# lizardfs/lizardfs

Hardware: NVIDIA H100
Metric: GiB/s encoded+CRC (ec(8,2), 64 MiB chunks) (higher is better)
Workload: dtype u8

## Files before the change

lizardfs_b200/csrc/fused.cu:

```cuda
#include <cuda.h>
#include <cuda_runtime.h>

#include <algorithm>
#include <cmath>
#include <numeric>
#include <cstdlib>
#include <cstring>
#include <memory>
#include <mutex>

#include "engine_internal.h"
#include "fused_kernel.cuh"
#include "convert_kernel.cuh"
#include "bs_recover_kernel.cuh"
#include "check_kernel.cuh"
#include "slices_kernel.cuh"
#include "recover_slices_kernel.cuh"
#include "host_math.h"

using namespace lzd;

typedef CUresult (*EncodeTiledFn)(CUtensorMap *, CUtensorMapDataType, cuuint32_t, void *, const cuuint64_t *, const cuuint64_t *,
                                  const cuuint32_t *, const cuuint32_t *, CUtensorMapInterleave, CUtensorMapSwizzle,
                                  CUtensorMapL2promotion, CUtensorMapFloatOOBfill);
// ... 62 lines not shown

static void set_raid6_pair(CoefPlanes *w, int x0, int x1) {
	const uint8_t g0 = gf_pow2(x0);
	coef_planes_set(w[0], g0);
	coef_planes_set(w[1], lz::gf_inv_host(g0 ^ gf_pow2(x1)));
}

static void elim3_constants(int x0, int x1, int x2, uint8_t c[6]) {
	const uint8_t A = gf_pow2(x0), pp = A ^ gf_pow2(x1), qq = A ^ gf_pow2(x2);
	c[0] = lz::gf_inv_host(lz::gf_mul_host(qq, pp ^ qq));
	c[1] = lz::gf_mul_host(pp, c[0]);
	c[2] = lz::gf_inv_host(pp);
	c[3] = lz::gf_mul_host(qq, c[2]);
	c[4] = A;
	c[5] = lz::gf_mul_host(A, A);
}

template <class... P, class... A>
static int launch(lzgpu_ctx *ctx, void (*kernel)(P...), const lzgpu_launch_geometry &geo, int per_sm, uint64_t units, cudaStream_t st,
                  const A &...args) {
	const int grid = persistent_grid(ctx, units, per_sm, geo);
	kernel<<<grid, geo.threads, geo.smem_bytes, st>>>(args...);
	CUDA_TRY(cudaGetLastError());
	ctx->stats.kernel_launches++;
	return LZGPU_OK;
}

template <class F>
static int set_smem(F *kernel, int bytes) {
	CUDA_TRY(cudaFuncSetAttribute(kernel, cudaFuncAttributeMaxDynamicSharedMemorySize, bytes));
	return LZGPU_OK;
}

using EncodeKernel = void (*)(CUtensorMap, FusedParams);
struct EncodeKernelEntry {
	int m;
	bool generic, striped, split, bs;
	uint32_t k, g;
	EncodeKernel fn;
	EncodeKernel narrow;
};
template <int M, bool GENERIC, int KT = 0, int GT = 0, bool STRIPED = false, bool SPLIT = false>
static EncodeKernelEntry encoder() {
	EncodeKernelEntry k{M, GENERIC, STRIPED, SPLIT, false, KT, GT, fused_stream_kernel<M, GENERIC, KT, GT, 64, STRIPED, SPLIT>, nullptr};
	if constexpr (GENERIC) k.narrow = fused_stream_kernel<M, GENERIC, KT, GT, 64, STRIPED, SPLIT, 1>;
	return k;
}
template <int M, int KT = 0, int GT = 0, bool STRIPED = false>
static EncodeKernelEntry bitsliced() {
	return {M, false, STRIPED, false, true, KT, GT, fused_stream_kernel<M, false, KT, GT, 64, STRIPED, false, 8>, nullptr};
}
static const EncodeKernelEntry kEncoders[] = {
	encoder<0, false>(), encoder<1, false>(), encoder<2, false>(), encoder<3, false>(), encoder<4, false>(),
	encoder<1, true>(), encoder<2, true>(), encoder<3, true>(), encoder<4, true>(),
	encoder<1, false, 0, 0, false, true>(), encoder<2, false, 0, 0, false, true>(), encoder<3, false, 0, 0, false, true>(),
	encoder<4, false, 0, 0, false, true>(), encoder<4, true, 0, 0, false, true>(),
	encoder<1, false, 0, 0, true>(), encoder<2, false, 0, 0, true>(), encoder<3, false, 0, 0, true>(), encoder<4, false, 0, 0, true>(),
	encoder<4, true, 0, 0, true>(),
	encoder<2, false, 8, 7>(),
	encoder<1, false, 2, 32>(),
	encoder<1, false, 3, 20>(),
	encoder<2, false, 3, 16>(),
	encoder<2, false, 4, 12>(),
	encoder<2, false, 6, 9>(),
	encoder<3, false, 5, 8>(),
	encoder<3, false, 6, 8>(),
	encoder<4, false, 8, 8>(),
	encoder<3, false, 8, 6>(),
	encoder<1, false, 4, 16>(),
	encoder<2, false, 5, 10>(),
	encoder<2, false, 10, 5>(),
	encoder<3, false, 4, 8>(),
	encoder<4, false, 10, 6>(),
	encoder<4, false, 12, 5>(),
	encoder<4, false, 6, 8>(),
	encoder<4, false, 4, 8>(),
	encoder<2, false, 8, 7, true>(), encoder<1, false, 2, 32, true>(), encoder<1, false, 3, 20, true>(), encoder<2, false, 3, 16, true>(),
	encoder<3, false, 5, 8, true>(), encoder<4, false, 8, 8, true>(),
	bitsliced<3>(), bitsliced<4>(), bitsliced<3, 0, 0, true>(), bitsliced<4, 0, 0, true>(),
	bitsliced<4, 8, 8>(), bitsliced<4, 10, 6>(), bitsliced<4, 12, 5>(), bitsliced<4, 6, 8>(), bitsliced<4, 4, 8>(),
	bitsliced<3, 8, 8>(), bitsliced<3, 9, 6>(), bitsliced<3, 10, 6>(), bitsliced<3, 12, 5>(), bitsliced<4, 8, 8, true>(),
};

static const EncodeKernelEntry *find_encoder(int M, bool generic, uint32_t K, uint32_t G, bool striped, bool split, bool bs) {
	const EncodeKernelEntry *runtime_k = nullptr;
	for (const EncodeKernelEntry &k : kEncoders) {
		if (k.m != M || k.generic != generic || k.striped != striped || k.split != split || k.bs != bs) continue;
		if (k.k == K && k.g == G) return &k;
		if (k.k == 0) runtime_k = &k;
	}
	return runtime_k;
}

using RecoverKernel = void (*)(TmapArray, RecoverParams);
struct RecoverKernelEntry {
	int kernel;
	uint32_t e, kt;
	bool first_e, wide;
	RecoverKernel fn;
};
template <int GEO, int E, int KT, int R0 = -1, int R1 = -1>
static RecoverKernelEntry recoverer() {
	constexpr int kernel = GEO == 2 ? LZGPU_KERNEL_RECOVER_GEO2 : GEO == 1 ? LZGPU_KERNEL_RECOVER_GEO1 : LZGPU_KERNEL_RECOVER_GEO0;
	return {kernel, E, KT, R0 == 0, false, fused_recover_kernel<E, KT, R0, R1, 64, GEO>};
}
template <int E, bool WIDE>
static RecoverKernelEntry direct() {
	return {LZGPU_KERNEL_RECOVER_DIRECT, E, 0, false, WIDE, fused_recover_kernel<E, 0, kRecoverDirect, -1, 64, 2, WIDE ? direct_wide_words(E) : 1>};
}
static const RecoverKernelEntry kRecoverers[] = {
	recoverer<0, 1, 8, 0>(), recoverer<1, 1, 8, 0>(), recoverer<2, 1, 8, 0>(),
	recoverer<0, 1, 0, 0>(), recoverer<1, 1, 0, 0>(), recoverer<2, 1, 0, 0>(),
	recoverer<0, 1, 0>(), recoverer<1, 1, 0>(), recoverer<2, 1, 0>(),
	recoverer<0, 2, 8, 0, 1>(), recoverer<1, 2, 8, 0, 1>(), recoverer<2, 2, 8, 0, 1>(),
	recoverer<0, 2, 0, 0, 1>(), recoverer<1, 2, 0, 0, 1>(), recoverer<2, 2, 0, 0, 1>(),
	recoverer<0, 2, 0>(), recoverer<1, 2, 0>(), recoverer<2, 2, 0>(),
	recoverer<0, 3, 0, 0, 1>(), recoverer<2, 3, 0, 0, 1>(), recoverer<0, 3, 0>(), recoverer<2, 3, 0>(),
	recoverer<0, 4, 0, 0, 1>(), recoverer<2, 4, 0, 0, 1>(), recoverer<0, 4, 0>(), recoverer<2, 4, 0>(),
	recoverer<2, 1, 3, 0>(), recoverer<2, 2, 3, 0, 1>(), recoverer<2, 2, 4, 0, 1>(), recoverer<2, 2, 5, 0, 1>(),
	recoverer<2, 3, 5, 0, 1>(), recoverer<2, 2, 6, 0, 1>(), recoverer<2, 3, 6, 0, 1>(),
// ... 128 lines not shown
}

void lz_fused_destroy(lzgpu_ctx *ctx) {
	if (ctx->fused && ctx->fused->d_sm_ctr) cudaFree(ctx->fused->d_sm_ctr);
	delete ctx->fused;
	ctx->fused = nullptr;
}

extern "C" int lzgpu_debug_last_launch(lzgpu_ctx *ctx, uint32_t *grid, uint32_t *units) {
	if (!ctx || !ctx->fused || !grid || !units) return LZGPU_ERR_ARG;
	std::lock_guard<std::mutex> lock(ctx->fused->last_mu);
	*grid = ctx->fused->last_geo.grid;
	*units = ctx->fused->last_geo.units;
	return LZGPU_OK;
}

extern "C" int lzgpu_debug_last_geometry(lzgpu_ctx *ctx, lzgpu_launch_geometry *out) {
	if (!ctx || !ctx->fused || !out) return LZGPU_ERR_ARG;
	std::lock_guard<std::mutex> lock(ctx->fused->last_mu);
	*out = ctx->fused->last_geo;
	return LZGPU_OK;
}

static CUresult make_tensor_map(const FusedState *fs, CUtensorMap *map, const void *base, uint64_t rows_per_chunk, uint64_t n_chunks,
                                uint64_t chunk_stride, uint32_t box_rows) {
	const cuuint64_t dims[3] = {static_cast<cuuint64_t>(kRowBytes), rows_per_chunk, n_chunks};
	const cuuint64_t strides[2] = {static_cast<cuuint64_t>(kRowBytes), chunk_stride ? chunk_stride : rows_per_chunk * kRowBytes};
	const cuuint32_t box[3] = {kStepBytes, box_rows, 1};
	const cuuint32_t estr[3] = {1, 1, 1};
	return fs->encode_tiled(map, CU_TENSOR_MAP_DATA_TYPE_UINT8, 3, const_cast<void *>(base), dims, strides, box, estr, CU_TENSOR_MAP_INTERLEAVE_NONE,
	                        CU_TENSOR_MAP_SWIZZLE_128B, static_cast<CUtensorMapL2promotion>(fs->promo), CU_TENSOR_MAP_FLOAT_OOB_FILL_NONE);
}

static int fused_run(lzgpu_ctx *ctx, int M, bool generic, const uint8_t *coef_rows, uint32_t K, uint32_t n_chunks, uint32_t nb,
                     const void *d_data, size_t chunk_stride, void *d_parity, size_t parity_stride, void *d_crc, size_t crc_stride,
                     cudaStream_t st, void *const *split_out = nullptr, size_t split_stride = 0, uint32_t crc_row_base = 0, bool skip_data_crc = false,
                     int striped_policy = -2 ) {
	FusedState *fs = ctx->fused;
	const int spol = split_out ? 0 : (striped_policy == -2 ? fs->striped : striped_policy);
	FusedPlan pl;
	if (!split_out && fused_bitslice(M, generic, fs->bitslice, K))
		pl = fused_plan(M, generic, K, n_chunks, nb, chunk_stride, std::min(fs->max_smem, fs->bs_smem_cap), 64, spol, true, fs->bs_max_stages, fs->bs_max_gf_warps);
	if (!pl.ok) pl = fused_plan(M, generic, K, n_chunks, nb, chunk_stride, std::min(fs->max_smem, fused_smem_cap(M, generic, 64)), 64, spol);
	if (!pl.ok || (reinterpret_cast<uintptr_t>(d_data) % 16)) return LZGPU_NOT_HANDLED;
	const uint32_t G = pl.G;
	const bool flat = pl.mode == 1u, striped = pl.mode == 2u;
	FusedParams p{};
	p.parity = static_cast<uint8_t *>(d_parity);
	p.crc = static_cast<uint32_t *>(d_crc);
	p.tables = ctx->d_crc_tables;
	p.parity_stride = parity_stride;
	p.crc_stride = crc_stride;
	p.n_chunks = n_chunks;
	p.nb = nb;
	p.pb = pl.pb;
	p.K = K;
	p.G = G;
	p.n_stages = pl.n_stages;
	p.flat = pl.mode;
	p.flat_magic = (1ull << 40) / p.pb + 1;
	p.units_per_chunk = pl.units_per_chunk;
	p.total_units = pl.total_units;
	std::memcpy(p.qmult, fs->qmult, sizeof(p.qmult));
	p.zconst = lz::crc_of_zeros(LZGPU_BLOCK_SIZE);
	p.probe = fs->probe;
	p.evict_first = static_cast<uint32_t>(fs->evict_first);
	p.crc_row_base = crc_row_base;
	p.skip_data_crc = skip_data_crc ? 1u : 0u;
	if (generic) {
		for (int r = 0; r < M; ++r)
			for (uint32_t j = 0; j < K; ++j) {
				coef_planes_set(p.coef[r * 32 + j], coef_rows[r * K + j]);
			}
	}
	const uint64_t map_rows = flat ? static_cast<uint64_t>(n_chunks) * nb * 4 : static_cast<uint64_t>(nb) * 4, map_chunks = flat ? 1 : n_chunks;
	const uint64_t map_stride = flat ? 0 : chunk_stride;
	const uint32_t box_rows = striped ? K * 4 : G * K * 4;
	CUtensorMap map;
	const CUresult r = make_tensor_map(fs, &map, d_data, map_rows, map_chunks, map_stride, box_rows);
	if (r != CUDA_SUCCESS) {
		lz_set_error("cuTensorMapEncodeTiled failed with CUresult %d (rows/chunk %llu, chunks %llu, stride %llu, box rows %u)", static_cast<int>(r),
		             static_cast<unsigned long long>(map_rows), static_cast<unsigned long long>(map_chunks), static_cast<unsigned long long>(map_stride), box_rows);
		return LZGPU_ERR_CUDA;
	}
	if (split_out) {
		if (striped || (split_stride % 16)) return LZGPU_NOT_HANDLED;
		for (uint32_t j = 0; j < K; ++j) p.data_out[j] = static_cast<uint8_t *>(split_out[j]);
		for (int r = 0; r < M; ++r) p.par_out[r] = static_cast<uint8_t *>(split_out[K + r]);
		p.part_out_stride = split_stride;
	}
	const EncodeKernelEntry *k = find_encoder(M, generic, K, G, striped, split_out != nullptr, pl.bs);
	if (!k) return LZGPU_NOT_HANDLED;
	const lzgpu_launch_geometry geo = launch_geo(pl.bs ? LZGPU_KERNEL_ENCODE_BITSLICE : LZGPU_KERNEL_ENCODE, pl.threads, G, pl.n_stages,
	                                             pl.bs ? (16 * G + 31) / 32 : 0, pl.smem);
	const EncodeKernel fn = k->narrow && fused_generic_item_words(G) == 1 ? k->narrow : k->fn;
	return launch(ctx, fn, geo, fused_ctas_per_sm(M, generic, 64, pl.bs), p.total_units, st, map, p);
}

int lz_fused_encode(lzgpu_ctx *ctx, const lzgpu_goal *goal, uint32_t n_chunks, uint32_t nb, const void *d_data, size_t chunk_stride,
                    void *d_parity, size_t parity_stride, void *d_crc, size_t crc_stride, cudaStream_t st) {
	FusedState *fs = ctx->fused;
	if (!fs || fs->disabled) return LZGPU_NOT_HANDLED;
	const int K = goal->k, M = goal->m;
	if (lz::uses_cauchy(K, M)) {
		if (fs->cauchy_encode_off) return LZGPU_NOT_HANDLED;
		uint8_t gen[LZGPU_MAX_PARTS * LZGPU_MAX_DATA];
		lz::rs_generator(K, M, gen);
		if (M == 4) return fused_run(ctx, 4, true, gen + K * K, K, n_chunks, nb, d_data, chunk_stride, d_parity, parity_stride, d_crc, crc_stride, st);
		const uint32_t pb = (nb + K - 1) / K;
		for (int rows : {4, M % 4})
			if (rows && !fused_plan(rows, true, K, n_chunks, nb, chunk_stride, std::min(fs->max_smem, fused_smem_cap(rows, true, 64)), 64, 0).ok) return LZGPU_NOT_HANDLED;
		if (reinterpret_cast<uintptr_t>(d_data) % 16) return LZGPU_NOT_HANDLED;
		for (int r0 = 0; r0 < M; r0 += 4) {
			int rc = fused_run(ctx, std::min(4, M - r0), true, gen + (K + r0) * K, K, n_chunks, nb, d_data, chunk_stride,
			                   static_cast<uint8_t *>(d_parity) + static_cast<size_t>(r0) * pb * LZGPU_BLOCK_SIZE, parity_stride, d_crc, crc_stride, st, nullptr, 0,
			                   static_cast<uint32_t>(r0), r0 > 0, 0);
			if (rc != LZGPU_OK) return rc == LZGPU_NOT_HANDLED ? LZGPU_ERR_CUDA : rc;
		}
		return LZGPU_OK;
	}
	if (M > 4) return LZGPU_NOT_HANDLED;
	int rc = fused_run(ctx, M, false, nullptr, K, n_chunks, nb, d_data, chunk_stride, d_parity, parity_stride, d_crc, crc_stride, st);
	if (rc == LZGPU_NOT_HANDLED && goal->kind == LZGPU_KIND_EC) {
		uint8_t gen[LZGPU_MAX_PARTS * LZGPU_MAX_DATA];
		lz::rs_generator(K, M, gen);
		rc = fused_run(ctx, M, true, gen + K * K, K, n_chunks, nb, d_data, chunk_stride, d_parity, parity_stride, d_crc, crc_stride, st, nullptr, 0, 0, false, 0);
	}
	return rc;
}
// ... 462 lines not shown
```

lizardfs_b200/csrc/fused_kernel.cuh:

```cuda
#pragma once
#include <cuda.h>

#include "bitslice.cuh"
#include "device_math.cuh"
#include "fused_plan.h"

namespace lzd {

#ifdef LZ_ENABLE_PROBE
#define LZ_PROBE(bit) (p.probe & (bit))
#else
#define LZ_PROBE(bit) 0
#endif

#ifdef LZ_ALL_LANES_ARRIVE
#define LZ_RING_ARRIVERS 32u
#define LZ_RING_LANE(lane) true
#else
#define LZ_RING_ARRIVERS 1u
#define LZ_RING_LANE(lane) ((lane) == 0)
#endif

struct FusedParams {
	uint8_t *parity;
// ... 45 lines not shown
	return false;
}
__device__ __forceinline__ void mbar_expect_tx(uint32_t bar, uint32_t bytes) {
	asm volatile("mbarrier.arrive.expect_tx.shared::cta.b64 _, [%0], %1;" ::"r"(bar), "r"(bytes) : "memory");
}
__device__ __forceinline__ void mbar_wait(uint32_t addr, uint32_t parity) {
	uint32_t done;
	do {
		asm volatile(
		    "{\n\t.reg .pred p;\n\t"
		    "mbarrier.try_wait.parity.shared::cta.b64 p, [%1], %2, %3;\n\t"
		    "selp.u32 %0, 1, 0, p;\n\t}"
		    : "=r"(done)
		    : "r"(addr), "r"(parity), "r"(0x989680u)
		    : "memory");
	} while (!done);
}
__device__ __forceinline__ void tma_load_3d_evict_first(uint32_t smem_dst, const CUtensorMap *map, int c0, int c1, int c2, uint32_t bar) {
	uint64_t policy;
	asm volatile("createpolicy.fractional.L2::evict_first.b64 %0, 1.0;" : "=l"(policy));
	asm volatile(
	    "cp.async.bulk.tensor.3d.shared::cluster.global.tile.mbarrier::complete_tx::bytes.L2::cache_hint [%0], [%1, {%2, %3, %4}], [%5], %6;" ::"r"(
	        smem_dst),
	    "l"(reinterpret_cast<uint64_t>(map)), "r"(c0), "r"(c1), "r"(c2), "r"(bar), "l"(policy)
	    : "memory");
}
__device__ __forceinline__ void tma_load_3d(uint32_t smem_dst, const CUtensorMap *map, int c0, int c1, int c2, uint32_t bar) {
	asm volatile(
	    "cp.async.bulk.tensor.3d.shared::cluster.global.tile.mbarrier::complete_tx::bytes [%0], [%1, {%2, %3, %4}], [%5];" ::"r"(
	        smem_dst),
	    "l"(reinterpret_cast<uint64_t>(map)), "r"(c0), "r"(c1), "r"(c2), "r"(bar)
	    : "memory");
}

template <int FW>
struct FoldSpec;
template <>
struct FoldSpec<64> {
	static constexpr int deg = 53, nlag = 9;
	__host__ __device__ static constexpr int lag(int t) { return t == 0 ? 15 : t == 1 ? 17 : t == 2 ? 20 : t == 3 ? 23 : t == 4 ? 26 : t == 5 ? 28 : t == 6 ? 46 : t == 7 ? 50 : 53; }
};

__device__ __forceinline__ uint4 lds128(uint32_t addr) {
	uint4 v;
	asm volatile("ld.shared.v4.u32 {%0,%1,%2,%3}, [%4];" : "=r"(v.x), "=r"(v.y), "=r"(v.z), "=r"(v.w) : "r"(addr));
	return v;
}
__device__ __forceinline__ void sts128(uint32_t addr, const uint4 &v) {
	asm volatile("st.shared.v4.u32 [%0], {%1,%2,%3,%4};" ::"r"(addr), "r"(v.x), "r"(v.y), "r"(v.z), "r"(v.w) : "memory");
}

template <int W>
__device__ __forceinline__ void lds_item(uint32_t addr, uint32_t (&v)[W]) {
	if constexpr (W == 4) asm volatile("ld.shared.v4.u32 {%0,%1,%2,%3}, [%4];" : "=r"(v[0]), "=r"(v[1]), "=r"(v[2]), "=r"(v[3]) : "r"(addr));
	else if constexpr (W == 2) asm volatile("ld.shared.v2.u32 {%0,%1}, [%2];" : "=r"(v[0]), "=r"(v[1]) : "r"(addr));
	else asm volatile("ld.shared.u32 %0, [%1];" : "=r"(v[0]) : "r"(addr));
}
template <int W>
__device__ __forceinline__ void sts_item(uint32_t addr, const uint32_t (&v)[W]) {
	if constexpr (W == 4) asm volatile("st.shared.v4.u32 [%0], {%1,%2,%3,%4};" ::"r"(addr), "r"(v[0]), "r"(v[1]), "r"(v[2]), "r"(v[3]) : "memory");
	else if constexpr (W == 2) asm volatile("st.shared.v2.u32 [%0], {%1,%2};" ::"r"(addr), "r"(v[0]), "r"(v[1]) : "memory");
	else asm volatile("st.shared.u32 [%0], %1;" ::"r"(addr), "r"(v[0]) : "memory");
}
template <int W>
__device__ __forceinline__ void stg_item(void *p, const uint32_t (&v)[W]) {
	if constexpr (W == 4) asm volatile(LZ_STG ".v4.u32 [%0], {%1,%2,%3,%4};" ::"l"(p), "r"(v[0]), "r"(v[1]), "r"(v[2]), "r"(v[3]) : "memory");
// ... 25 lines not shown
		win[S & (FW - 1)] = acc;
	}
}

template <int FW, bool AUX = true>
__device__ __forceinline__ void fold_step(uint32_t (&win)[FW], FoldAux &aux, int base, uint32_t row_addr_swz) {
#pragma unroll
	for (int c = 0; c < 8; ++c) {
		const uint4 v = lds128(row_addr_swz ^ (c << 4));
		fold_word<FW, AUX>(win, aux, base + 4 * c + 0, v.x);
		fold_word<FW, AUX>(win, aux, base + 4 * c + 1, v.y);
		fold_word<FW, AUX>(win, aux, base + 4 * c + 2, v.z);
		fold_word<FW, AUX>(win, aux, base + 4 * c + 3, v.w);
	}
}

template <int FW>
__device__ __forceinline__ uint32_t fold_finish(uint32_t (&win)[FW], const uint32_t *tab) {
	constexpr int deg = FoldSpec<FW>::deg;
#pragma unroll
	for (int j = 0; j < deg; ++j) {
		uint32_t acc = 0;
#pragma unroll
		for (int t = 0; t < FoldSpec<FW>::nlag; ++t)
			if (FoldSpec<FW>::lag(t) > j) acc ^= win[(j - FoldSpec<FW>::lag(t)) & (FW - 1)];
		win[j] = acc;
	}
	uint32_t st = 0;
#pragma unroll
	for (int j = 0; j < deg; ++j) st = crc_step_word_ldg(st, win[j], tab);
	return st;
}

template <int M, bool GENERIC, int KT, int GT, int FW, bool STRIPED = false, bool SPLIT = false, int W = fused_item_words(M, GENERIC)>
__global__ void __launch_bounds__(fused_threads(M, GENERIC, W == 8), fused_ctas_per_sm(M, GENERIC, FW, W == 8))
fused_stream_kernel(const __grid_constant__ CUtensorMap tmap, const FusedParams p) {
	constexpr int kNSTc = fused_nst(FW, M, GENERIC, W == 8), kNPST = fused_npst(FW, M, GENERIC);
	const uint32_t kNST = (W == 8) ? p.n_stages : static_cast<uint32_t>(kNSTc);
	constexpr int NT = fused_threads(M, GENERIC, W == 8);
	constexpr int PC = (M == 0) ? 0 : (GENERIC ? M : M - 1);
	constexpr int P0 = GENERIC ? 0 : 1;
	constexpr bool BS = W == 8;
	static_assert(!BS || ((M == 3 || M == 4) && !GENERIC && !SPLIT && FW == 64), "bit-sliced items: three or four Vandermonde rows, plain encode");

	extern __shared__ __align__(1024) uint8_t smem[];
	const uint32_t sbase = smem_u32(smem);
	const uint32_t K = KT ? KT : p.K, G = GT ? GT : p.G;
	const uint32_t ROWS = G * K * 4;
	const uint32_t PROWS = G * PC * 4;
	const uint32_t stage_bytes = ROWS * kStepBytes;
	const uint32_t pstage_bytes = (PROWS * kStepBytes + 1023u) & ~1023u;
	const uint32_t pstage0 = sbase + kNST * stage_bytes;
	const uint32_t misc = pstage0 + kNPST * pstage_bytes;
	const uint32_t a_blk = misc;
	const uint32_t a_full = misc + 520, a_empty = a_full + 8 * kNST, a_pfull = a_empty + 8 * kNST, a_pempty = a_pfull + 8 * kNPST;

	const uint32_t tid = threadIdx.x;
	const uint32_t warp = tid >> 5, lane = tid & 31;
	constexpr uint32_t CPI = 32 / W;
	const uint32_t n_items = 4 * CPI * G * (M > 0 ? 1 : 0);
	const uint32_t n_gf_warps = (min(n_items, (uint32_t)NT) + 31) / 32;
	const uint32_t bs_gf_warps = BS ? n_gf_warps : 0, bs_gf_warp0 = NT / 32 - bs_gf_warps;
	const uint32_t first_pwarp = ROWS / 32, last_pwarp = PROWS ? (ROWS + PROWS - 1) / 32 : 0;
	const uint32_t n_stage_warps = BS ? bs_gf_warps + (ROWS + 31) / 32 : max((ROWS + 31) / 32, n_gf_warps);

	const uint32_t my_units = blockIdx.x < p.total_units ? (p.total_units - blockIdx.x + gridDim.x - 1) / gridDim.x : 0;
	const uint32_t total_steps = my_units * kStepsPerUnit;

	auto issue_load = [&](uint32_t c, uint32_t gi, uint32_t step, uint32_t st) {
		mbar_expect_tx(a_full + 8 * st, stage_bytes);
		if (p.evict_first)
			tma_load_3d_evict_first(sbase + st * stage_bytes, &tmap, static_cast<int>(step * kStepBytes), static_cast<int>(gi * ROWS),
			                        static_cast<int>(c), a_full + 8 * st);
		else
			tma_load_3d(sbase + st * stage_bytes, &tmap, static_cast<int>(step * kStepBytes), static_cast<int>(gi * ROWS), static_cast<int>(c),
			            a_full + 8 * st);
	};

	auto issue_striped = [&](uint32_t unit, uint32_t step, uint32_t st, uint32_t first_g, uint32_t g_step) {
		const uint32_t s0 = unit * G;
		const uint32_t n_valid = min(G, p.n_chunks * p.pb - s0);
		const uint32_t stripe_bytes = K * 4 * kStepBytes;
		if (first_g == 0) mbar_expect_tx(a_full + 8 * st, n_valid * stripe_bytes);
		for (uint32_t g = first_g; g < n_valid; g += g_step) {
// ... 11 lines not shown
			s_out = sg - cc * p.pb;
		} else {
			c_out = unit_c;
			s_out = sg;
		}
	};
	const uint32_t stripes_total = p.flat ? p.n_chunks * p.pb : p.pb;

	if (tid == 0) {
		for (uint32_t s = 0; s < kNST; ++s) {
			mbar_init(a_full + 8 * s, 1);
			mbar_init(a_empty + 8 * s, n_stage_warps);
		}
		for (int s = 0; s < kNPST; ++s) {
			mbar_init(a_pfull + 8 * s, (n_gf_warps ? n_gf_warps : 1) * LZ_RING_ARRIVERS);
			mbar_init(a_pempty + 8 * s, (PROWS ? (last_pwarp - first_pwarp + 1) : 1) * LZ_RING_ARRIVERS);
		}
		asm volatile("fence.mbarrier_init.release.cluster;" ::: "memory");
		if (total_steps)
			for (uint32_t g0 = 0; g0 < kNST; ++g0) {
				if (STRIPED) issue_striped(blockIdx.x, g0, g0, 0, 1);
				else issue_load(blockIdx.x / p.units_per_chunk, blockIdx.x % p.units_per_chunk, g0, g0);
			}
	}
	__syncthreads();

	const uint32_t cw = warp;
	const uint32_t vt = tid;
	const bool is_data_row = vt < ROWS;
	const bool is_parity_row = vt >= ROWS && vt < ROWS + PROWS;
	const bool has_stream = is_data_row || is_parity_row;
	const uint32_t prow = vt - ROWS;
	const uint32_t my_row = is_data_row ? vt : prow;
	const uint32_t row_addr0 = ((is_data_row ? sbase : pstage0) + my_row * kStepBytes) ^ ((my_row & 7) << 4);
	const uint32_t row_stride = is_data_row ? stage_bytes : pstage_bytes;
	const bool warp_has_items = !BS && cw < n_gf_warps;
	const bool warp_has_prow = PROWS && cw >= first_pwarp && cw <= last_pwarp;
	const bool warp_reads_stage = BS ? cw < (ROWS + 31) / 32 : cw < n_stage_warps;

	if constexpr (BS) {
		if (cw >= bs_gf_warp0) {
			uint32_t it = 0, st = 0, ph = 0, pst = 0, pph = 0;
			const uint32_t item = tid - 32 * bs_gf_warp0;
			const bool has_item = item < n_items;
			const uint32_t col = item & 7, h = (item >> 3) & 1, g = item >> 4;
			const uint32_t rbase = g * K * 4 + h;
			const uint32_t a_even0 = (rbase * kStepBytes) ^ ((col ^ (rbase & 7)) << 4);
			for (uint32_t unit = blockIdx.x; unit < p.total_units; unit += gridDim.x) {
				const uint32_t c = unit / p.units_per_chunk, gi = unit % p.units_per_chunk;
				const uint32_t stripe0 = gi * G;
				const uint32_t next_unit = unit + gridDim.x;
				const uint32_t next_c = next_unit / p.units_per_chunk, next_gi = next_unit % p.units_per_chunk;
				const uint32_t sg = stripe0 + g;
				uint32_t pc = 0, stripe = 0;
				const bool live = has_item && sg < stripes_total;
				if (live) locate(sg, c, pc, stripe);
				uint8_t *const dst0 = p.parity + pc * p.parity_stride + (static_cast<unsigned long long>(stripe) << 16) + (h << 14) + col * 16;
				const unsigned long long part_bytes = static_cast<unsigned long long>(p.pb) * 65536ull;
				for (int step = 0; step < kStepsPerUnit; ++step) {
					const uint32_t stage = sbase + st * stage_bytes;
					const uint32_t pstage = pstage0 + pst * pstage_bytes;
					mbar_wait(a_full + 8 * st, ph);
					if (!LZ_PROBE(2)) {
						mbar_wait(a_pempty + 8 * pst, pph ^ 1);
						if (has_item) {
							BsRows<BS ? M : 4> rows4;
							bs_rows_clear(rows4);
// ... 35 lines not shown
						if (__shfl_sync(0xffffffffu, refill, 0)) {
							asm volatile("fence.proxy.async.shared::cta;" ::: "memory");
							if (step + kNST < kStepsPerUnit) issue_striped(unit, step + kNST, st, lane, 32);
							else issue_striped(next_unit, step + kNST - kStepsPerUnit, st, lane, 32);
						}
					} else if (lane == 0) {
						if (mbar_arrive_is_last(a_empty + 8 * st) && it + kNST < total_steps) {
							asm volatile("fence.proxy.async.shared::cta;" ::: "memory");
							if (step + kNST < kStepsPerUnit) issue_load(c, gi, step + kNST, st);
							else issue_load(next_c, next_gi, step + kNST - kStepsPerUnit, st);
						}
					}
					++it;
					if (++st == kNST) { st = 0; ph ^= 1; }
					if (++pst == kNPST) { pst = 0; pph ^= 1; }
				}
			}
			return;
		}
	}

	uint32_t win[FW];
	FoldAux aux;
	uint32_t it = 0;
	uint32_t st = 0, ph = 0;
	uint32_t pst = 0, pph = 0;
	uint32_t unit_parity = 0;

	for (uint32_t unit = blockIdx.x; unit < p.total_units; unit += gridDim.x, unit_parity ^= 1) {
		const uint32_t c = unit / p.units_per_chunk, gi = unit % p.units_per_chunk;
		const uint32_t stripe0 = gi * G;
		const uint32_t next_unit = unit + gridDim.x;
		const uint32_t next_c = next_unit / p.units_per_chunk, next_gi = next_unit % p.units_per_chunk;
#pragma unroll
		for (int i = 0; i < FW; ++i) win[i] = 0;
#pragma unroll
		for (int i = 0; i < 32; ++i) aux.y[i] = 0;

		for (int step0 = 0; step0 < kStepsPerUnit; step0 += FW / 32) {
#pragma unroll
			for (int sub = 0; sub < FW / 32; ++sub) {
				const int step = step0 + sub;
				const uint32_t stage = sbase + st * stage_bytes;
				const uint32_t pstage = pstage0 + pst * pstage_bytes;
				if (warp_reads_stage) mbar_wait(a_full + 8 * st, ph);

				if (!BS && M > 0 && warp_has_items && !LZ_PROBE(2)) {
					if (PC > 0) mbar_wait(a_pempty + 8 * pst, pph ^ 1);
					for (uint32_t item = vt; item < n_items; item += NT) {
						const uint32_t col = item % CPI, q = (item / CPI) & 3, g = item / (4 * CPI);
						const uint32_t c16 = (col * W) >> 2, sub = ((col * W) & 3) << 2;
						uint32_t acc[M > 0 ? M : 1][W];
#pragma unroll
						for (int r = 0; r < M; ++r)
#pragma unroll
							for (int w = 0; w < W; ++w) acc[r][w] = 0;
						const uint32_t rbase = g * K * 4 + q;
						const uint32_t sg = stripe0 + g;
						uint32_t pc = 0, stripe = 0;
						if (sg < stripes_total) locate(sg, c, pc, stripe);
						const unsigned long long in_part = (static_cast<unsigned long long>(stripe) << 16) + (q << 14) + step * kStepBytes + col * (4 * W);
						const uint32_t a_even = ((stage + rbase * kStepBytes) ^ ((c16 ^ (rbase & 7)) << 4)) + sub;
						const uint32_t a_odd = ((stage + rbase * kStepBytes) ^ ((c16 ^ ((rbase & 7) ^ 4)) << 4)) + sub;
#pragma unroll
						for (int j = static_cast<int>(K) - 1; j >= 0; --j) {
							uint32_t v[W];
							lds_item<W>(((j & 1) ? a_odd : a_even) + 4u * j * kStepBytes, v);
							if (SPLIT) {
								uint8_t *dp = p.data_out[j];
								if (dp && sg < stripes_total) stg_item<W>(dp + pc * p.part_out_stride + in_part, v);
							}
							if (GENERIC) {
#pragma unroll
								for (int r = 0; r < M; ++r) {
									const CoefPlanes &cp = p.coef[r * 32 + j];
#pragma unroll
									for (int w = 0; w < W; ++w) acc[r][w] = gf_mac<6>(acc[r][w], v[w], cp);
								}
							} else {
#pragma unroll
								for (int r = 0; r < M; ++r) {
#pragma unroll
									for (int w = 0; w < W; ++w) {
										const uint32_t a = acc[r][w], d = v[w];
										acc[r][w] = r == 0 ? (a ^ d) : r == 1 ? gf_x2_add(a, d) : r == 2 ? gf_x4_add(a, d) : gf_x8_add(a, d);
									}
								}
							}
						}
						if (sg < stripes_total && !LZ_PROBE(8)) {
							if (SPLIT) {
#pragma unroll
								for (int r = 0; r < M; ++r)
									if (p.par_out[r]) stg_item<W>(p.par_out[r] + pc * p.part_out_stride + in_part, acc[r]);
							} else {
								uint8_t *dst = p.parity + pc * p.parity_stride + in_part;
#pragma unroll
								for (int r = 0; r < M; ++r) stg_item<W>(dst + static_cast<unsigned long long>(r) * p.pb * 65536ull, acc[r]);
							}
						}
#pragma unroll
						for (int r = P0; r < M; ++r) {
							const uint32_t pr = (g * PC + (r - P0)) * 4 + q;
							sts_item<W>(((pstage + pr * kStepBytes) ^ ((c16 ^ (pr & 7)) << 4)) + sub, acc[r]);
						}
					}
					if (PC > 0) {
						__syncwarp();
						if (LZ_RING_LANE(lane)) mbar_arrive(a_pfull + 8 * pst);
					}
				}

				if (PC > 0 && warp_has_prow && !LZ_PROBE(2)) mbar_wait(a_pfull + 8 * pst, pph);
				if (has_stream && !(GENERIC && is_data_row && p.skip_data_crc) && !LZ_PROBE(4)) {
					const uint32_t rowp = row_addr0 + (is_data_row ? st : pst) * row_stride;
					fold_step<FW, (NT * fused_ctas_per_sm(M, GENERIC, FW, BS) <= 512)>(win, aux, sub * 32, rowp);
				}
				__syncwarp();
				if (STRIPED) {
					uint32_t refill = 0;
					if (lane == 0) refill = warp_reads_stage && mbar_arrive_is_last(a_empty + 8 * st) && it + kNST < total_steps;
					if (__shfl_sync(0xffffffffu, refill, 0)) {
						asm volatile("fence.proxy.async.shared::cta;" ::: "memory");
						if (step + kNST < kStepsPerUnit) issue_striped(unit, step + kNST, st, lane, 32);
						else issue_striped(next_unit, step + kNST - kStepsPerUnit, st, lane, 32);
					}
				} else if (lane == 0) {
					if (warp_reads_stage && mbar_arrive_is_last(a_empty + 8 * st) && it + kNST < total_steps) {
						asm volatile("fence.proxy.async.shared::cta;" ::: "memory");
						if (step + kNST < kStepsPerUnit) issue_load(c, gi, step + kNST, st);
						else issue_load(next_c, next_gi, step + kNST - kStepsPerUnit, st);
					}
				}
				if (PC > 0 && warp_has_prow && !LZ_PROBE(2) && LZ_RING_LANE(lane)) mbar_arrive(a_pempty + 8 * pst);
				++it;
				if (++st == kNST) { st = 0; ph ^= 1; }
				if (++pst == kNPST) { pst = 0; pph ^= 1; }
			}
		}

		uint32_t lin = 0;
		if (has_stream) lin = crc_mulmod(fold_finish<FW>(win, p.tables), p.qmult[my_row & 3]);
		lin ^= __shfl_xor_sync(0xffffffffu, lin, 1);
		lin ^= __shfl_xor_sync(0xffffffffu, lin, 2);
		const uint32_t blk = a_blk + unit_parity * 256;
		if (is_data_row && (vt & 3) == 0) {
			const uint32_t bl = vt >> 2;
			if (M > 0 && !GENERIC) asm volatile("st.shared.u32 [%0], %1;" ::"r"(blk + (vt & ~3u)), "r"(lin) : "memory");
			const uint32_t sg = stripe0 + bl / K;
			uint32_t bc, bs;
			locate(sg, c, bc, bs);
			const uint32_t b = bs * K + bl % K;
			if (sg < stripes_total && b < p.nb && !(GENERIC && p.skip_data_crc)) p.crc[bc * p.crc_stride + b] = lin ^ p.zconst;
		}
		if (is_parity_row && (prow & 3) == 0) {
			constexpr uint32_t PCD = PC ? PC : 1;
			const uint32_t g = (prow >> 2) / PCD, r = P0 + (prow >> 2) % PCD;
			const uint32_t sg = stripe0 + g;
			uint32_t pc, stripe;
			locate(sg, c, pc, stripe);
			if (sg < stripes_total) p.crc[pc * p.crc_stride + p.nb + (p.crc_row_base + r) * p.pb + stripe] = lin ^ p.zconst;
		}
		if (M > 0 && !GENERIC) {
			asm volatile("bar.sync 1, %0;" ::"r"(NT - 32 * static_cast<int>(bs_gf_warps)) : "memory");
			if (vt < G) {
				uint32_t x = 0;
				for (uint32_t j = 0; j < K; ++j) {
					uint32_t t;
					asm volatile("ld.shared.u32 %0, [%1];" : "=r"(t) : "r"(blk + 4 * (vt * K + j)));
					x ^= t;
				}
				const uint32_t sg = stripe0 + vt;
				uint32_t pc, stripe;
				locate(sg, c, pc, stripe);
				if (sg < stripes_total) p.crc[pc * p.crc_stride + p.nb + stripe] = x ^ p.zconst;
			}
		}
	}
}

struct TmapArray {
	CUtensorMap m[32];
};

struct RecoverParams {
	uint8_t *out[4];
	uint8_t *image;
	const uint32_t *stored[32];
	const uint32_t *tables;
	unsigned long long *first_bad;
	unsigned long long out_stride, image_stride;
	uint32_t n_chunks, nb, pb, K, G, units_per_chunk, total_units;
	uint32_t e;
	uint32_t n_stages;
	uint32_t raid6_dbl;
	uint32_t elim3_dbl;
	uint8_t slot_of_data[32];
	uint8_t erased_idx[4];
	uint8_t par_slot[4], par_row[4];
	uint8_t part_id[32];
	uint32_t qmult[4];
	uint32_t zconst;
	CoefPlanes w[16];
	uint8_t data_of_slot[32];
	CoefPlanes rw[4 * 32];
};

constexpr int kRecoverDirect = -2;

#pragma nv_diag_suppress 128
template <int E, int KT, int R0, int R1, int kRecoverFW, int GEO = 0, int W = recover_item_words(E, GEO)>
// ... 258 lines not shown
```

lizardfs_b200/csrc/fused_plan.h:

```cpp
#pragma once
#include <cstddef>
#include <cstdint>

#include "lzgpu.h"

#ifndef __CUDACC__
#define LZ_HD
#else
#define LZ_HD __host__ __device__
#endif

namespace lzd {

constexpr int kStepBytes = 128;
constexpr int kRowBytes = 16384;
constexpr int kStepsPerUnit = kRowBytes / kStepBytes;
constexpr int kConsumers = 288;
constexpr int kFusedThreads = kConsumers;
constexpr int kMaxRows = 256;
constexpr int kMaxParityRows = 128;
constexpr int kSmemCap = 113 * 1024;

#ifndef LZ_T2
#define LZ_T2 256
// ... 43 lines not shown
	return fused_smem_bytes_n(rows, prows, fused_nst(fw, m, generic, bs), fused_npst(fw, m, generic));
}
#ifndef LZ_BS_MAX_STAGES
#define LZ_BS_MAX_STAGES 4
#endif

#ifndef LZ_GCAP
#define LZ_GCAP 1
#endif
#ifndef LZ_BS_MAX_GF_WARPS
#define LZ_BS_MAX_GF_WARPS 4
#endif
inline uint32_t pick_group(uint32_t K, uint32_t PC, int max_smem_per_cta, int fw, uint32_t threads, int m, bool generic, bool bs = false,
                           int bs_max_gf_warps = LZ_BS_MAX_GF_WARPS) {
	uint32_t best = 0;
	const uint32_t items_per_stripe = bs ? 16u : 128u / static_cast<uint32_t>(fused_item_words(m, generic));
	for (uint32_t g = 1; g <= 64; ++g) {
		const uint32_t gf_warps = bs ? (g * items_per_stripe + 31) / 32 : 0;
		if (bs ? gf_warps > static_cast<uint32_t>(bs_max_gf_warps) : (LZ_GCAP && (threads > 288 || m >= 3) && m > 0 && best && g * items_per_stripe > threads)) break;
		const uint32_t rows = g * K * 4, prows = g * PC * 4;
		if (rows > kMaxRows || rows + prows > threads - 32 * gf_warps || prows > kMaxParityRows || g * K > 64) break;
		if (rows % 8) continue;
		if (fused_smem_bytes(rows, prows, fw, m, generic, bs) > static_cast<size_t>(max_smem_per_cta)) break;
		best = g;
	}
	return best;
}

struct FusedPlan {
	uint32_t G = 0, pb = 0, mode = 0, units_per_chunk = 0, total_units = 0, threads = 0, rows = 0, prows = 0, n_stages = 0;
	size_t smem = 0;
	bool ok = false;
	bool bs = false;
};

inline FusedPlan fused_plan(int M, bool generic, uint32_t K, uint32_t n_chunks, uint32_t nb, size_t chunk_stride, int smem_cap, int fw,
                            int striped_policy, bool bs = false, int bs_max_stages = LZ_BS_MAX_STAGES, int bs_max_gf_warps = LZ_BS_MAX_GF_WARPS) {
	FusedPlan pl;
	const uint32_t PC = M == 0 ? 0 : (generic ? M : M - 1);
	const int mm = M;
	pl.threads = static_cast<uint32_t>(fused_threads(mm, generic, bs));
	pl.bs = bs;
	pl.G = pick_group(K, PC, smem_cap, fw, pl.threads, mm, generic, bs, bs_max_gf_warps);
	if (pl.G == 0 || (chunk_stride % 16)) return pl;
	const uint32_t G = pl.G;
	pl.pb = (nb + K - 1) / K;
	const bool flat = n_chunks > 1 && chunk_stride == static_cast<size_t>(nb) * 65536u && nb % K == 0 &&
	                  static_cast<uint64_t>(n_chunks) * pl.pb < (1ull << 31) && static_cast<uint64_t>(n_chunks) * nb * 4 < (1ull << 31);
	pl.mode = flat ? 1u : 0u;
	if (!flat && M > 0 && static_cast<uint64_t>(n_chunks) * pl.pb < (1ull << 31) && static_cast<uint64_t>(nb) * 4 < (1ull << 31)) {
		const uint64_t per_chunk_slots = static_cast<uint64_t>((pl.pb + G - 1) / G) * G * n_chunks;
		const uint64_t stripes = static_cast<uint64_t>(n_chunks) * pl.pb;
		const bool wasteful = per_chunk_slots * 100 > stripes * 112;
		if (striped_policy == 1 || (striped_policy < 0 && wasteful)) pl.mode = 2u;
	}
	uint64_t total;
	if (pl.mode != 0) {
		pl.units_per_chunk = static_cast<uint32_t>((static_cast<uint64_t>(n_chunks) * pl.pb + G - 1) / G);
		total = pl.units_per_chunk;
	} else {
		pl.units_per_chunk = (pl.pb + G - 1) / G;
		total = static_cast<uint64_t>(pl.units_per_chunk) * n_chunks;
	}
	if (total > 0x7fffffffull) return pl;
	pl.total_units = static_cast<uint32_t>(total);
	pl.rows = G * K * 4;
	pl.prows = G * PC * 4;
	pl.n_stages = static_cast<uint32_t>(fused_nst(fw, mm, generic, bs));
	const size_t npst = fused_npst(fw, mm, generic);
	if (bs)
		while (static_cast<int>(pl.n_stages) < bs_max_stages && fused_smem_bytes_n(pl.rows, pl.prows, pl.n_stages + 1, npst) <= static_cast<size_t>(smem_cap)) ++pl.n_stages;
	pl.smem = fused_smem_bytes_n(pl.rows, pl.prows, pl.n_stages, npst);
	pl.ok = true;
	return pl;
}

constexpr int kConvertThreads = 256;
constexpr int kConvertNPST = 4;

struct ConvertPlan {
	bool ok = false;
	uint32_t G = 0, T = 0, region_rows = 0, n_stages = 0, n_workers = 0;
	uint32_t e = 0;
	uint8_t erased[2] = {0, 0};
	size_t smem = 0;
};

inline ConvertPlan convert_plan(int Ks, int Ms, bool src_cauchy, int Kd, int Md, bool dst_cauchy, const uint8_t *available, int max_smem) {
	ConvertPlan pl;
	if (src_cauchy || dst_cauchy || Md < 1 || Md > 3 || Ks < 1 || Ks > 32 || Kd < 1 || Kd > 32) return pl;
	int n_used = 0, n_par = 0;
	bool present[32] = {false};
	for (int i = 0; i < Ks + Ms && n_used < Ks; ++i) {
		if (!available[i]) continue;
		++n_used;
		if (i < Ks) present[i] = true;
		else if (i == Ks + n_par && n_par < 2) ++n_par;
		else return pl;
	}
	if (n_used < Ks) return pl;
	uint32_t e = 0;
	for (int j = 0; j < Ks; ++j)
		if (!present[j]) {
			if (e >= 2) return pl;
			pl.erased[e++] = static_cast<uint8_t>(j);
// ... 314 lines not shown
```

Baseline: 2201.

## Stage M=2 parity through shared-memory ring and store via TMA with evict-first

For two-row Vandermonde encodes, parity accumulators are written into a doubled shared-memory parity stage instead of being stored directly to global memory. The last parity warp then issues 4D TMA bulk tensor stores with an L2 evict_first hint, covering two steps at a time, and releases the slots once the bulk reads complete. This replaces scattered per-thread global stores with coalesced asynchronous bulk writes and keeps parity out of L2. In exchange it doubles parity shared memory, adds proxy fences and wait_group stalls, and serialises the store issue onto one lane.

New measurement: 2220 (median of 6 runs). No clear change (+0.9%).

```diff
diff --git a/lizardfs_b200/csrc/fused.cu b/lizardfs_b200/csrc/fused.cu
--- a/lizardfs_b200/csrc/fused.cu
+++ b/lizardfs_b200/csrc/fused.cu
@@ -118,23 +118,27 @@
 	return LZGPU_OK;
 }
 
-using EncodeKernel = void (*)(CUtensorMap, FusedParams);
+using EncodeKernel = void (*)(CUtensorMap, CUtensorMap, FusedParams);
 struct EncodeKernelEntry {
 	int m;
-	bool generic, striped, split, bs;
+	bool generic, striped, split, bs, ring;
 	uint32_t k, g;
 	EncodeKernel fn;
 	EncodeKernel narrow;
 };
 template <int M, bool GENERIC, int KT = 0, int GT = 0, bool STRIPED = false, bool SPLIT = false>
 static EncodeKernelEntry encoder() {
-	EncodeKernelEntry k{M, GENERIC, STRIPED, SPLIT, false, KT, GT, fused_stream_kernel<M, GENERIC, KT, GT, 64, STRIPED, SPLIT>, nullptr};
+	EncodeKernelEntry k{M, GENERIC, STRIPED, SPLIT, false, false, KT, GT, fused_stream_kernel<M, GENERIC, KT, GT, 64, STRIPED, SPLIT>, nullptr};
 	if constexpr (GENERIC) k.narrow = fused_stream_kernel<M, GENERIC, KT, GT, 64, STRIPED, SPLIT, 1>;
 	return k;
 }
 template <int M, int KT = 0, int GT = 0, bool STRIPED = false>
 static EncodeKernelEntry bitsliced() {
-	return {M, false, STRIPED, false, true, KT, GT, fused_stream_kernel<M, false, KT, GT, 64, STRIPED, false, 8>, nullptr};
+	return {M, false, STRIPED, false, true, false, KT, GT, fused_stream_kernel<M, false, KT, GT, 64, STRIPED, false, 8>, nullptr};
+}
+template <int KT = 0, int GT = 0>
+static EncodeKernelEntry ringed() {
+	return {2, false, false, false, false, true, KT, GT, fused_stream_kernel<2, false, KT, GT, 64, false, false, 4, true>, nullptr};
 }
 static const EncodeKernelEntry kEncoders[] = {
 	encoder<0, false>(), encoder<1, false>(), encoder<2, false>(), encoder<3, false>(), encoder<4, false>(),
@@ -166,12 +170,13 @@
 	bitsliced<3>(), bitsliced<4>(), bitsliced<3, 0, 0, true>(), bitsliced<4, 0, 0, true>(),
 	bitsliced<4, 8, 8>(), bitsliced<4, 10, 6>(), bitsliced<4, 12, 5>(), bitsliced<4, 6, 8>(), bitsliced<4, 4, 8>(),
 	bitsliced<3, 8, 8>(), bitsliced<3, 9, 6>(), bitsliced<3, 10, 6>(), bitsliced<3, 12, 5>(), bitsliced<4, 8, 8, true>(),
+	ringed<>(), ringed<8, 7>(), ringed<10, 5>(),
 };
 
-static const EncodeKernelEntry *find_encoder(int M, bool generic, uint32_t K, uint32_t G, bool striped, bool split, bool bs) {
+static const EncodeKernelEntry *find_encoder(int M, bool generic, uint32_t K, uint32_t G, bool striped, bool split, bool bs, bool ring) {
 	const EncodeKernelEntry *runtime_k = nullptr;
 	for (const EncodeKernelEntry &k : kEncoders) {
-		if (k.m != M || k.generic != generic || k.striped != striped || k.split != split || k.bs != bs) continue;
+		if (k.m != M || k.generic != generic || k.striped != striped || k.split != split || k.bs != bs || k.ring != ring) continue;
 		if (k.k == K && k.g == G) return &k;
 		if (k.k == 0) runtime_k = &k;
 	}
@@ -366,6 +371,16 @@
 	                        CU_TENSOR_MAP_SWIZZLE_128B, static_cast<CUtensorMapL2promotion>(fs->promo), CU_TENSOR_MAP_FLOAT_OOB_FILL_NONE);
 }
 
+static CUresult make_parity_map(const FusedState *fs, CUtensorMap *map, void *base, uint32_t pb, uint64_t n_chunks, uint64_t parity_stride) {
+	const uint64_t part_bytes = static_cast<uint64_t>(pb) * LZGPU_BLOCK_SIZE;
+	const cuuint64_t dims[4] = {static_cast<cuuint64_t>(kRowBytes), static_cast<cuuint64_t>(pb) * 4, 2, n_chunks};
+	const cuuint64_t strides[3] = {static_cast<cuuint64_t>(kRowBytes), part_bytes, n_chunks > 1 ? parity_stride : 2 * part_bytes};
+	const cuuint32_t box[4] = {kStepBytes, 4, 2, 1};
+	const cuuint32_t estr[4] = {1, 1, 1, 1};
+	return fs->encode_tiled(map, CU_TENSOR_MAP_DATA_TYPE_UINT8, 4, base, dims, strides, box, estr, CU_TENSOR_MAP_INTERLEAVE_NONE,
+	                        CU_TENSOR_MAP_SWIZZLE_128B, CU_TENSOR_MAP_L2_PROMOTION_NONE, CU_TENSOR_MAP_FLOAT_OOB_FILL_NONE);
+}
+
 static int fused_run(lzgpu_ctx *ctx, int M, bool generic, const uint8_t *coef_rows, uint32_t K, uint32_t n_chunks, uint32_t nb,
                      const void *d_data, size_t chunk_stride, void *d_parity, size_t parity_stride, void *d_crc, size_t crc_stride,
                      cudaStream_t st, void *const *split_out = nullptr, size_t split_stride = 0, uint32_t crc_row_base = 0, bool skip_data_crc = false,
@@ -377,6 +392,10 @@
 		pl = fused_plan(M, generic, K, n_chunks, nb, chunk_stride, std::min(fs->max_smem, fs->bs_smem_cap), 64, spol, true, fs->bs_max_stages, fs->bs_max_gf_warps);
 	if (!pl.ok) pl = fused_plan(M, generic, K, n_chunks, nb, chunk_stride, std::min(fs->max_smem, fused_smem_cap(M, generic, 64)), 64, spol);
 	if (!pl.ok || (reinterpret_cast<uintptr_t>(d_data) % 16)) return LZGPU_NOT_HANDLED;
+	if (pl.ring && (split_out || (reinterpret_cast<uintptr_t>(d_parity) % 16) || (parity_stride % 16))) {
+		pl.ring = false;
+		pl.smem = fused_smem_bytes_n(pl.rows, pl.prows, pl.n_stages, fused_npst(64, M, generic));
+	}
 	const uint32_t G = pl.G;
 	const bool flat = pl.mode == 1u, striped = pl.mode == 2u;
 	FusedParams p{};
@@ -423,12 +442,21 @@
 		for (int r = 0; r < M; ++r) p.par_out[r] = static_cast<uint8_t *>(split_out[K + r]);
 		p.part_out_stride = split_stride;
 	}
-	const EncodeKernelEntry *k = find_encoder(M, generic, K, G, striped, split_out != nullptr, pl.bs);
+	CUtensorMap pmap = map;
+	if (pl.ring) {
+		const CUresult rp = make_parity_map(fs, &pmap, d_parity, pl.pb, n_chunks, parity_stride);
+		if (rp != CUDA_SUCCESS) {
+			lz_set_error("cuTensorMapEncodeTiled failed with CUresult %d for the parity map (pb %u, chunks %u, stride %llu)", static_cast<int>(rp), pl.pb,
+			             n_chunks, static_cast<unsigned long long>(parity_stride));
+			return LZGPU_ERR_CUDA;
+		}
+	}
+	const EncodeKernelEntry *k = find_encoder(M, generic, K, G, striped, split_out != nullptr, pl.bs, pl.ring);
 	if (!k) return LZGPU_NOT_HANDLED;
 	const lzgpu_launch_geometry geo = launch_geo(pl.bs ? LZGPU_KERNEL_ENCODE_BITSLICE : LZGPU_KERNEL_ENCODE, pl.threads, G, pl.n_stages,
 	                                             pl.bs ? (16 * G + 31) / 32 : 0, pl.smem);
 	const EncodeKernel fn = k->narrow && fused_generic_item_words(G) == 1 ? k->narrow : k->fn;
-	return launch(ctx, fn, geo, fused_ctas_per_sm(M, generic, 64, pl.bs), p.total_units, st, map, p);
+	return launch(ctx, fn, geo, fused_ctas_per_sm(M, generic, 64, pl.bs), p.total_units, st, map, pmap, p);
 }
 
 int lz_fused_encode(lzgpu_ctx *ctx, const lzgpu_goal *goal, uint32_t n_chunks, uint32_t nb, const void *d_data, size_t chunk_stride,
diff --git a/lizardfs_b200/csrc/fused_kernel.cuh b/lizardfs_b200/csrc/fused_kernel.cuh
--- a/lizardfs_b200/csrc/fused_kernel.cuh
+++ b/lizardfs_b200/csrc/fused_kernel.cuh
@@ -101,6 +101,16 @@
 	    "l"(reinterpret_cast<uint64_t>(map)), "r"(c0), "r"(c1), "r"(c2), "r"(bar)
 	    : "memory");
 }
+__device__ __forceinline__ void tma_store_4d_evict_first(const CUtensorMap *map, int c0, int c1, int c2, int c3, uint32_t smem_src) {
+	uint64_t policy;
+	asm volatile("createpolicy.fractional.L2::evict_first.b64 %0, 1.0;" : "=l"(policy));
+	asm volatile("cp.async.bulk.tensor.4d.global.shared::cta.bulk_group.L2::cache_hint [%0, {%1, %2, %3, %4}], [%5], %6;" ::"l"(reinterpret_cast<uint64_t>(map)),
+	             "r"(c0), "r"(c1), "r"(c2), "r"(c3), "r"(smem_src), "l"(policy)
+	             : "memory");
+}
+__device__ __forceinline__ void bulk_commit() { asm volatile("cp.async.bulk.commit_group;" ::: "memory"); }
+__device__ __forceinline__ void bulk_wait_read_all() { asm volatile("cp.async.bulk.wait_group.read 0;" ::: "memory"); }
+__device__ __forceinline__ void bulk_wait_all() { asm volatile("cp.async.bulk.wait_group 0;" ::: "memory"); }
 
 template <int FW>
 struct FoldSpec;
@@ -192,9 +202,10 @@
 	return st;
 }
 
-template <int M, bool GENERIC, int KT, int GT, int FW, bool STRIPED = false, bool SPLIT = false, int W = fused_item_words(M, GENERIC)>
+template <int M, bool GENERIC, int KT, int GT, int FW, bool STRIPED = false, bool SPLIT = false, int W = fused_item_words(M, GENERIC),
+          bool RING = false>
 __global__ void __launch_bounds__(fused_threads(M, GENERIC, W == 8), fused_ctas_per_sm(M, GENERIC, FW, W == 8))
-fused_stream_kernel(const __grid_constant__ CUtensorMap tmap, const FusedParams p) {
+fused_stream_kernel(const __grid_constant__ CUtensorMap tmap, const __grid_constant__ CUtensorMap pmap, const FusedParams p) {
 	constexpr int kNSTc = fused_nst(FW, M, GENERIC, W == 8), kNPST = fused_npst(FW, M, GENERIC);
 	const uint32_t kNST = (W == 8) ? p.n_stages : static_cast<uint32_t>(kNSTc);
 	constexpr int NT = fused_threads(M, GENERIC, W == 8);
@@ -202,6 +213,7 @@
 	constexpr int P0 = GENERIC ? 0 : 1;
 	constexpr bool BS = W == 8;
 	static_assert(!BS || ((M == 3 || M == 4) && !GENERIC && !SPLIT && FW == 64), "bit-sliced items: three or four Vandermonde rows, plain encode");
+	static_assert(!RING || (M == 2 && !GENERIC && !STRIPED && !SPLIT && W == 4 && kNPST % 2 == 0), "parity through the ring: two Vandermonde rows, plain encode, slot pairs");
 
 	extern __shared__ __align__(1024) uint8_t smem[];
 	const uint32_t sbase = smem_u32(smem);
@@ -209,7 +221,7 @@
 	const uint32_t ROWS = G * K * 4;
 	const uint32_t PROWS = G * PC * 4;
 	const uint32_t stage_bytes = ROWS * kStepBytes;
-	const uint32_t pstage_bytes = (PROWS * kStepBytes + 1023u) & ~1023u;
+	const uint32_t pstage_bytes = ((RING ? 2 : 1) * PROWS * kStepBytes + 1023u) & ~1023u;
 	const uint32_t pstage0 = sbase + kNST * stage_bytes;
 	const uint32_t misc = pstage0 + kNPST * pstage_bytes;
 	const uint32_t a_blk = misc;
@@ -287,7 +299,8 @@
 	const bool has_stream = is_data_row || is_parity_row;
 	const uint32_t prow = vt - ROWS;
 	const uint32_t my_row = is_data_row ? vt : prow;
-	const uint32_t row_addr0 = ((is_data_row ? sbase : pstage0) + my_row * kStepBytes) ^ ((my_row & 7) << 4);
+	const uint32_t slot_row = is_data_row ? vt : RING ? 2 * (prow & ~3u) + 4 + (prow & 3) : prow;
+	const uint32_t row_addr0 = ((is_data_row ? sbase : pstage0) + slot_row * kStepBytes) ^ ((slot_row & 7) << 4);
 	const uint32_t row_stride = is_data_row ? stage_bytes : pstage_bytes;
 	const bool warp_has_items = !BS && cw < n_gf_warps;
 	const bool warp_has_prow = PROWS && cw >= first_pwarp && cw <= last_pwarp;
@@ -389,6 +402,9 @@
 		const uint32_t stripe0 = gi * G;
 		const uint32_t next_unit = unit + gridDim.x;
 		const uint32_t next_c = next_unit / p.units_per_chunk, next_gi = next_unit % p.units_per_chunk;
+		uint32_t ring_c0 = c, ring_s0 = stripe0;
+		if (RING && p.flat) locate(stripe0, c, ring_c0, ring_s0);
+		const uint32_t ring_n = min(G, stripes_total - stripe0);
 #pragma unroll
 		for (int i = 0; i < FW; ++i) win[i] = 0;
 #pragma unroll
@@ -445,24 +461,33 @@
 								}
 							}
 						}
-						if (sg < stripes_total && !LZ_PROBE(8)) {
-							if (SPLIT) {
-#pragma unroll
-								for (int r = 0; r < M; ++r)
-									if (p.par_out[r]) stg_item<W>(p.par_out[r] + pc * p.part_out_stride + in_part, acc[r]);
-							} else {
-								uint8_t *dst = p.parity + pc * p.parity_stride + in_part;
-#pragma unroll
-								for (int r = 0; r < M; ++r) stg_item<W>(dst + static_cast<unsigned long long>(r) * p.pb * 65536ull, acc[r]);
-							}
-						}
-#pragma unroll
-						for (int r = P0; r < M; ++r) {
-							const uint32_t pr = (g * PC + (r - P0)) * 4 + q;
-							sts_item<W>(((pstage + pr * kStepBytes) ^ ((c16 ^ (pr & 7)) << 4)) + sub, acc[r]);
+						if constexpr (RING) {
+#pragma unroll
+							for (int r = 0; r < M; ++r) {
+								const uint32_t pr = g * 8 + r * 4 + q;
+								sts_item<W>(((pstage + pr * kStepBytes) ^ ((c16 ^ (pr & 7)) << 4)) + sub, acc[r]);
+							}
+						} else {
+							if (sg < stripes_total && !LZ_PROBE(8)) {
+								if (SPLIT) {
+#pragma unroll
+									for (int r = 0; r < M; ++r)
+										if (p.par_out[r]) stg_item<W>(p.par_out[r] + pc * p.part_out_stride + in_part, acc[r]);
+								} else {
+									uint8_t *dst = p.parity + pc * p.parity_stride + in_part;
+#pragma unroll
+									for (int r = 0; r < M; ++r) stg_item<W>(dst + static_cast<unsigned long long>(r) * p.pb * 65536ull, acc[r]);
+								}
+							}
+#pragma unroll
+							for (int r = P0; r < M; ++r) {
+								const uint32_t pr = (g * PC + (r - P0)) * 4 + q;
+								sts_item<W>(((pstage + pr * kStepBytes) ^ ((c16 ^ (pr & 7)) << 4)) + sub, acc[r]);
+							}
 						}
 					}
 					if (PC > 0) {
+						if (RING) asm volatile("fence.proxy.async.shared::cta;" ::: "memory");
 						__syncwarp();
 						if (LZ_RING_LANE(lane)) mbar_arrive(a_pfull + 8 * pst);
 					}
@@ -489,7 +514,32 @@
 						else issue_load(next_c, next_gi, step + kNST - kStepsPerUnit, st);
 					}
 				}
-				if (PC > 0 && warp_has_prow && !LZ_PROBE(2) && LZ_RING_LANE(lane)) mbar_arrive(a_pempty + 8 * pst);
+				if (PC > 0 && warp_has_prow && !LZ_PROBE(2)) {
+					if (RING && cw == last_pwarp) {
+						if (it & 1) {
+							if (lane == 0 && !LZ_PROBE(8)) {
+								asm volatile("fence.proxy.async.shared::cta;" ::: "memory");
+								const uint32_t prev = pstage0 + ((pst + kNPST - 1) % kNPST) * pstage_bytes;
+								uint32_t cc = ring_c0, s = ring_s0;
+								for (uint32_t g = 0; g < ring_n; ++g) {
+									tma_store_4d_evict_first(&pmap, (step - 1) * kStepBytes, static_cast<int>(4 * s), 0, static_cast<int>(cc), prev + g * 1024);
+									tma_store_4d_evict_first(&pmap, step * kStepBytes, static_cast<int>(4 * s), 0, static_cast<int>(cc), pstage + g * 1024);
+									if (++s == p.pb) { s = 0; ++cc; }
+								}
+								bulk_commit();
+							}
+						} else if (it >= 2) {
+							if (lane == 0) bulk_wait_read_all();
+							__syncwarp();
+							if (LZ_RING_LANE(lane)) {
+								mbar_arrive(a_pempty + 8 * ((pst + kNPST - 2) % kNPST));
+								mbar_arrive(a_pempty + 8 * ((pst + kNPST - 1) % kNPST));
+							}
+						}
+					} else if (LZ_RING_LANE(lane)) {
+						mbar_arrive(a_pempty + 8 * pst);
+					}
+				}
 				++it;
 				if (++st == kNST) { st = 0; ph ^= 1; }
 				if (++pst == kNPST) { pst = 0; pph ^= 1; }
@@ -534,6 +584,7 @@
 			}
 		}
 	}
+	if (RING && warp == last_pwarp && lane == 0) bulk_wait_all();
 }
 
 struct TmapArray {
diff --git a/lizardfs_b200/csrc/fused_plan.h b/lizardfs_b200/csrc/fused_plan.h
--- a/lizardfs_b200/csrc/fused_plan.h
+++ b/lizardfs_b200/csrc/fused_plan.h
@@ -99,6 +99,7 @@
 	size_t smem = 0;
 	bool ok = false;
 	bool bs = false;
+	bool ring = false;
 };
 
 inline FusedPlan fused_plan(int M, bool generic, uint32_t K, uint32_t n_chunks, uint32_t nb, size_t chunk_stride, int smem_cap, int fw,
@@ -138,6 +139,13 @@
 	if (bs)
 		while (static_cast<int>(pl.n_stages) < bs_max_stages && fused_smem_bytes_n(pl.rows, pl.prows, pl.n_stages + 1, npst) <= static_cast<size_t>(smem_cap)) ++pl.n_stages;
 	pl.smem = fused_smem_bytes_n(pl.rows, pl.prows, pl.n_stages, npst);
+	if (M == 2 && !generic && !bs && pl.mode != 2u) {
+		const size_t ring_smem = fused_smem_bytes_n(pl.rows, 2 * pl.prows, pl.n_stages, npst);
+		if (ring_smem <= static_cast<size_t>(smem_cap)) {
+			pl.ring = true;
+			pl.smem = ring_smem;
+		}
+	}
 	pl.ok = true;
 	return pl;
 }
```
